# migoox/genome-downsampler

Hardware: AMD Instinct MI355X
Metric: Mreads/s selected at target coverage M=100 (higher is better)
Workload: dtype u32

## Files before the change

genome-downsampler_amd/csrc/api/context.inc.hip:

```cpp
namespace {

thread_local char g_err[512] = "";

int fail(int code, const char* fmt, ...) {
    va_list ap;
    va_start(ap, fmt);
    vsnprintf(g_err, sizeof(g_err), fmt, ap);
    va_end(ap);
    return code;
}

#define HIP_TRY(expr)                                                                      \
    do {                                                                                   \
        hipError_t _e = (expr);                                                            \
        if (_e != hipSuccess)                                                              \
            return fail(_e == hipErrorOutOfMemory ? QMCP_ENOMEM : QMCP_EHIP, "%s: %s (%s:%d)", \
                        #expr, hipGetErrorString(_e), __FILE__, __LINE__);                 \
    } while (0)

struct DevBuf {
    void* p = nullptr;
    size_t cap = 0;
};

// ... 21 lines not shown
    bool pm = false;
    uint32_t range_shift = 0;
    uint32_t nu_filter = 0;
};

}

struct qmcp_hip_ctx {
    int device = 0;
    qmcp_hip_options opt = {};
    hipStream_t stream = nullptr;
    hipEvent_t ev[EV_COUNT] = {};
    hipEvent_t ev_in = nullptr;
    hipStream_t stream2 = nullptr;
    hipEvent_t ev_fork = nullptr;
    DevBuf roff, poff, stats, cstart, boff, ecnt, eoff, selend, spine, hist, spine2, hist2, specsnap, specflags;
    DevBuf keys[2], vals[2];
    DevBuf in_starts, in_ends, in_aux0, in_aux1, mask, cov, amp, next_head;
    DevBuf f_starts, f_ends, f_map, f_words, f_mask;
    DevBuf ranges;
    DevBuf rankamb;
    DevBuf pm_desc, pm_work;
    uint32_t nu_ell = 0;
    uint64_t nu_failed_n = 0, nu_failed_ltot = 0;
    uint32_t nu_failed_ell = 0, nu_failed_M = 0;
    uint64_t nu_need_n = 0, nu_need_ltot = 0;
    uint32_t nu_need_ell = 0, nu_need_M = 0, nu_need_rounds = 0;
    bool nu_deferred = false;
    DevBuf nu_exc, nu_nadj, nu_ce, nu_state, nu_sus, nu_ckpt, nu_prev;
    uint32_t* h_nu = nullptr;
// ... 216 lines not shown
```

genome-downsampler_amd/csrc/api/host_entries.inc.hip:

```cpp
int coverage_common(qmcp_hip_ctx* c, const uint32_t* starts, const uint32_t* ends, uint64_t n64,
                    const uint64_t* roff, const uint32_t* lengths, uint32_t n_contigs,
                    const uint64_t* keep_mask, uint32_t* cov_out) {
    TRY(use_device(c));
    if (c->pending) return fail(QMCP_EINVAL, "a solve is pending on this context (call qmcp_hip_solve_end)");
    if (n64 && (!starts || !ends)) return fail(QMCP_EINVAL, "null buffer");
    Problem pr;
    TRY(check_problem(roff, lengths, n_contigs, n64, pr));
    const uint32_t n = (uint32_t)pr.n, ltot = (uint32_t)pr.ltot;
    if (ltot == 0) return n ? fail(QMCP_EREAD, "reads given for zero-length contigs") : QMCP_OK;
    if (n == 0) {
        if (cov_out) std::memset(cov_out, 0, (size_t)ltot * sizeof(uint32_t));
        TRY(ensure(c, c->cov, (size_t)ltot * sizeof(uint32_t)));
        HIP_TRY(hipMemsetAsync(c->cov.p, 0, (size_t)ltot * sizeof(uint32_t), c->stream));
        HIP_TRY(hipStreamSynchronize(c->stream));
        return QMCP_OK;
    }
    TRY(ensure(c, c->in_starts, (size_t)n * 4));
    TRY(ensure(c, c->in_ends, (size_t)n * 4));
    HIP_TRY(hipMemcpyAsync(c->in_starts.p, starts, (size_t)n * 4, hipMemcpyHostToDevice, c->stream));
    HIP_TRY(hipMemcpyAsync(c->in_ends.p, ends, (size_t)n * 4, hipMemcpyHostToDevice, c->stream));
    const uint64_t* d_keep = nullptr;
    if (keep_mask) {
        const size_t words = (size_t)((n64 + 63) / 64);
        TRY(ensure(c, c->mask, words * 8));
// ... 134 lines not shown
        if (b->p) (void)hipFree(b->p);
    for (int i = 0; i < EV_COUNT; ++i)
        if (c->ev[i]) (void)hipEventDestroy(c->ev[i]);
    if (c->ev_in) (void)hipEventDestroy(c->ev_in);
    for (auto& sp : c->spans) { (void)hipEventDestroy(sp.a); (void)hipEventDestroy(sp.b); }
    for (hipEvent_t e : c->ev_pool) (void)hipEventDestroy(e);
    if (c->h_tables) (void)hipHostFree(c->h_tables);
    if (c->h_scalars) (void)hipHostFree(c->h_scalars);
    if (c->h_stage) (void)hipHostFree(c->h_stage);
    if (c->h_mask) (void)hipHostFree(c->h_mask);
    for (hipEvent_t e : c->stage_ev) (void)hipEventDestroy(e);
    for (hipEvent_t e : c->stage_done) (void)hipEventDestroy(e);
    for (hipStream_t st : c->stage_streams) (void)hipStreamDestroy(st);
    if (c->ev_fork) (void)hipEventDestroy(c->ev_fork);
    if (c->ev_head) (void)hipEventDestroy(c->ev_head);
    if (c->ev_done) (void)hipEventDestroy(c->ev_done);
    if (c->h_head) (void)hipHostFree(c->h_head);
    if (c->h_nu) (void)hipHostFree(c->h_nu);
    if (c->stream2) (void)hipStreamDestroy(c->stream2);
    if (c->stream) (void)hipStreamDestroy(c->stream);
    delete c;
}

int qmcp_hip_set_profiling(qmcp_hip_ctx* c, int enabled) {
    if (!c) return fail(QMCP_EINVAL, "null context");
    c->profiling = enabled == 2 ? 2 : (enabled != 0 ? 1 : 0);
    c->acc.clear();
    return QMCP_OK;
}

// ... 494 lines not shown
```

genome-downsampler_amd/csrc/api/near_uniform_route.inc.hip:

```cpp
constexpr uint32_t kNuRunInsApart = 2;
int near_uniform_tail(qmcp_hip_ctx* c, uint32_t min_span, uint32_t max_span, uint32_t max_load, uint32_t* d_iters, bool& done) {
    done = false;
    SolveRun& run = c->run;
    const Problem& pr = run.pr;
    qmcp_hip_stats& local = run.local;
    const uint32_t n = (uint32_t)pr.n, ltot = (uint32_t)pr.ltot, n_contigs = run.n_contigs, M = run.M;
    local.near_uniform_giveup = QMCP_NU_GIVEUP_NOT_TRIED;
    if (c->opt.near_uniform < 0) return QMCP_OK;
    const uint32_t ell = max_span;
    uint32_t longest = 0;
    for (uint32_t k = 0; k < n_contigs; ++k) longest = run.lengths[k] > longest ? run.lengths[k] : longest;
    const qmcp::NearUniformPlan plan = qmcp::plan_near_uniform(c->opt, n, ell, min_span, ltot, n_contigs, longest, M, run.may_rank);
    const bool stretches = plan.stretches, speculate = plan.speculate;
    const bool dbg = c->opt.near_uniform_debug == 1;
    if (dbg) fprintf(stderr, "[near] pm %d may_rank %d ell %u ev %d depth %.2f min_span %u filter %u\n", (int)run.pm,
                     (int)run.may_rank, ell, (int)qmcp::sweep_uniform_ev_supported(ell, M), plan.depth, min_span, run.nu_filter);
    if (!plan.tried) return QMCP_OK;
    if (c->nu_failed_n == run.n64 && c->nu_failed_ltot == pr.ltot && c->nu_failed_ell == ell && c->nu_failed_M == M) {
        local.near_uniform_giveup = QMCP_NU_GIVEUP_REMEMBERED;
        c->nu_ell = 0;
        return QMCP_OK;
    }
    hipStream_t st = c->stream;
    const uint32_t cap = nu_cap_for(n);
// ... 10 lines not shown
        HIP_TRY(hipStreamSynchronize(st));
        n_exc = n - c->h_nu[0];
        if (dbg) fprintf(stderr, "[near] reads of span %u: %u of %u, list holds %u\n", ell, c->h_nu[0], n, cap);
        if (n_exc > n / 10u) {
            c->nu_ell = 0;
            local.near_uniform_giveup = n_exc > n - n / 10u ? QMCP_NU_GIVEUP_LONGER_READS : QMCP_NU_GIVEUP_TOO_MANY;
            return QMCP_OK;
        }
        c->nu_ell = ell;
        if (run.pm) TRY(queue_pm_head(c, st, ell));
        else TRY(queue_rm_head(c, st, ell, true));
        uint32_t* d_max_load = (uint32_t*)c->ranges.p + 65540;
        HIP_TRY(hipMemcpyAsync(c->h_nu, d_max_load, sizeof(uint32_t), hipMemcpyDeviceToHost, st));
        HIP_TRY(hipMemcpyAsync(c->h_nu + 1, d_stats + 4, 2 * sizeof(uint32_t), hipMemcpyDeviceToHost, st));
        HIP_TRY(hipStreamSynchronize(st));
        max_load = c->h_nu[0];
        if (c->h_nu[1] != n_exc || c->h_nu[2] != 0) { c->nu_ell = 0; local.near_uniform_giveup = QMCP_NU_GIVEUP_TOO_MANY; return QMCP_OK; }
    }
    local.near_uniform_exceptions = n_exc;
    if (n_exc == 0 || n_exc > n / 10u || (uint64_t)max_load * kRankBalance > (uint64_t)n) {
        if (n_exc > n / 10u) c->nu_ell = 0;
        local.near_uniform_giveup = n_exc > n / 10u ? QMCP_NU_GIVEUP_TOO_MANY : n_exc == 0 ? QMCP_NU_GIVEUP_NOT_TRIED : QMCP_NU_GIVEUP_HEAVY_RANGE;
        return QMCP_OK;
    }
    if (!stretches) {
        TRY(ensure(c, c->evpk, qmcp::sweep_ev_pack_bytes(ltot, ell, n_contigs + 768)));
        TRY(ensure(c, c->evlast, qmcp::sweep_ev_last_bytes(ltot, ell, n_contigs + 768)));
    }
    const uint32_t* boff = (const uint32_t*)c->boff.p;
    const uint64_t* poff = (const uint64_t*)c->poff.p;
// ... 150 lines not shown
```

genome-downsampler_amd/csrc/api/solve_head.inc.hip:

```cpp
int queue_rm_head(qmcp_hip_ctx* c, hipStream_t s1, uint32_t filter, bool clear_mask);
int queue_pm_head(qmcp_hip_ctx* c, hipStream_t st, uint32_t filter);

bool pm_route_ok(const qmcp_hip_ctx* c, const uint64_t* roff, const Problem& pr, uint32_t shift) {
    if (c->opt.pass_major < 0) return false;
    const uint32_t n = (uint32_t)pr.n, ltot = (uint32_t)pr.ltot;
    if ((uint64_t)qmcp::pm_slots(n, ltot, shift) >= (1ull << 31)) return false;
    if (c->opt.pass_major > 0) return true;
    double slots = 0.0;
    for (uint32_t k = 0; k < pr.n_contigs; ++k) {
        const uint64_t reads = roff[k + 1] - roff[k];
        if (reads == 0 || pr.poff[k + 1] == pr.poff[k]) continue;
        const double ranges = (double)(((pr.poff[k + 1] - 1) >> shift) - (pr.poff[k] >> shift) + 1);
        const double passes = (double)reads / (double)qmcp::pm_pass() < 1.0 ? 1.0 : (double)reads / (double)qmcp::pm_pass();
        const double slice = (double)reads / (passes * ranges);
        slots += passes * ranges * std::ceil(slice / 64.0);
    }
    return slots <= 1.3 * ((double)n / 64.0);
}
int enqueue_head(qmcp_hip_ctx* c, const uint32_t* d_starts, const uint32_t* d_ends,
                 const uint64_t* roff, const uint32_t* lengths, uint32_t n_contigs, uint64_t n64,
                 uint32_t M, uint64_t* d_mask) {
    if (c->pending) return fail(QMCP_EINVAL, "a solve is already pending on this context (call qmcp_hip_solve_end)");
    c->pend_spiky = false;
    if (!c->h_scalars) HIP_TRY(hipHostMalloc((void**)&c->h_scalars, 16 * sizeof(unsigned long long), hipHostMallocDefault));
    SolveRun& run = c->run;
    run = SolveRun();
    run.d_starts = d_starts; run.d_ends = d_ends; run.roff = roff; run.lengths = lengths;
    run.n_contigs = n_contigs; run.n64 = n64; run.M = M; run.d_mask = d_mask;
    Problem& pr = run.pr;
    TRY(check_problem(roff, lengths, n_contigs, n64, pr));
    const uint32_t n = (uint32_t)pr.n;
    const uint32_t ltot = (uint32_t)pr.ltot;
    const size_t mask_words = (size_t)((n64 + 63) / 64);
    qmcp_hip_stats& local = run.local;
    std::memset(&local, 0, sizeof(local));
    local.n_reads = n64;
    local.n_contigs = n_contigs;
    local.total_length = pr.ltot;
// ... 146 lines not shown
        qmcp::launch_partition_level2(s1, c->keys[1].p, n, range_shift, d_seg_tables, (uint32_t*)c->hist.p,
                                      (uint32_t*)c->spine.p, (uint16_t*)c->keys[0].p,
                                      (uint32_t*)c->vals[0].p, d_range_start, d_max_load);
    }
    HIP_TRY(hipEventRecord(c->ev_fork, s1));
    {
        KernelSpan sp(c, "k_range_offsets");
        qmcp::launch_range_offsets(s1, (const uint16_t*)c->keys[0].p, d_range_start, range_shift, ltot,
                                   (uint32_t*)c->boff.p, (uint32_t*)c->stats.p + 3);
    }
    HIP_TRY(hipGetLastError());
    run.nu_filter = filter;
    return QMCP_OK;
}

int queue_pm_head(qmcp_hip_ctx* c, hipStream_t st, uint32_t filter) {
    SolveRun& run = c->run;
    const uint32_t n = (uint32_t)run.pr.n, ltot = (uint32_t)run.pr.ltot, n_contigs = run.n_contigs;
    uint32_t* d_stats = (uint32_t*)c->stats.p;
    static const uint32_t zeros[4] = {0u, 0u, 0u, 0u};
    HIP_TRY(hipMemcpyAsync(d_stats + 3, zeros, sizeof(zeros), hipMemcpyHostToDevice, st));
    uint32_t* d_range_start = (uint32_t*)c->ranges.p;
    uint32_t* d_max_load = d_range_start + 65540;
    {
        KernelSpan sp(c, "k_pm_prepare_sort", st);
        qmcp::launch_pm_prepare_sort(st, run.d_starts, run.d_ends, n, (const uint64_t*)c->roff.p, (const uint64_t*)c->poff.p,
                                     n_contigs, run.range_shift, ltot, (uint16_t*)c->keys[0].p, (uint16_t*)c->keys[1].p,
                                     (uint32_t*)c->hist2.p, (uint32_t*)c->hist.p,
                                     (uint32_t*)c->pm_work.p, d_stats, (unsigned long long*)run.d_mask, filter,
                                     filter ? (uint32_t*)c->nu_exc.p : nullptr, nu_cap_for(n),
                                     filter ? qmcp::nu_exc_counts((uint32_t*)c->nu_exc.p, nu_cap_for(n)) : nullptr);
    }
    HIP_TRY(hipGetLastError());
    HIP_TRY(hipEventRecord(c->ev[EV_PREP], st));
    {
        KernelSpan sp(c, "scan_radix_hist(3 kernels)", st);
        qmcp::launch_exclusive_scan(st, (const uint32_t*)c->hist2.p, 256u * qmcp::pm_pitch(n), (uint32_t*)c->hist2.p,
                                    (uint32_t*)c->spine2.p, true);
    }
    {
        KernelSpan sp(c, "k_pm_descr + k_pm_range_table", st);
        qmcp::launch_pm_descr(st, (const uint32_t*)c->hist2.p, (const uint32_t*)c->hist.p, n, ltot, run.range_shift,
                              (uint32_t*)c->pm_desc.p, (uint32_t*)c->pm_work.p, d_range_start, d_max_load);
    }
    HIP_TRY(hipEventRecord(c->ev_fork, st));
    {
        KernelSpan sp(c, "k_pm_offsets", st);
        qmcp::launch_pm_offsets(st, (const uint16_t*)c->keys[0].p, (const uint32_t*)c->pm_desc.p, (const uint32_t*)c->hist2.p, n,
                                d_range_start, run.range_shift, ltot, (uint32_t*)c->boff.p, d_stats + 3);
    }
    HIP_TRY(hipGetLastError());
    run.nu_filter = filter;
    return QMCP_OK;
}

void queue_pm_rank(qmcp_hip_ctx* c, hipStream_t st, const uint32_t* ev_sev, const uint32_t* ev_lastns, uint32_t ell) {
    SolveRun& run = c->run;
    const uint32_t n = (uint32_t)run.pr.n, ltot = (uint32_t)run.pr.ltot;
    const bool by_records = qmcp::rank_scratch_by_records(run.range_shift, ltot, n);
    const uint16_t* keys16 = (const uint16_t*)c->keys[0].p;
    const uint16_t* idx16 = (const uint16_t*)c->keys[1].p;
    const uint32_t* desc = (const uint32_t*)c->pm_desc.p;
    const uint32_t* Tp = (const uint32_t*)c->hist2.p;
    const uint32_t* range_start = (const uint32_t*)c->ranges.p;
    uint32_t* amb_count = (uint32_t*)c->pm_work.p + 512;
    unsigned long long* kept_total = (unsigned long long*)c->scalars.p;
    {
        KernelSpan sp(c, "k_pm_walk", st);
        qmcp::launch_pm_walk(st, keys16, idx16, desc, Tp, n, range_start, run.range_shift, ltot, (const uint32_t*)c->boff.p,
                             (const uint32_t*)c->selend.p, (unsigned long long*)run.d_mask, kept_total, c->rankamb.p, by_records,
                             amb_count, ev_sev, ev_lastns, (const uint64_t*)c->poff.p, run.n_contigs, ell);
    }
    KernelSpan sp(c, "k_pm_settle", st);
    qmcp::launch_pm_settle(st, keys16, idx16, desc, Tp, n, range_start, run.range_shift, ltot, c->rankamb.p, by_records,
                           amb_count, (unsigned long long*)run.d_mask, kept_total);
}
```

genome-downsampler_amd/csrc/api/solve_tail.inc.hip:

```cpp
int enqueue_tail(qmcp_hip_ctx* c) {
    SolveRun& run = c->run;
    const Problem& pr = run.pr;
    qmcp_hip_stats& local = run.local;
    const uint32_t n = (uint32_t)pr.n, ltot = (uint32_t)pr.ltot, n_contigs = run.n_contigs, M = run.M;
    const uint64_t n64 = run.n64;
    const uint32_t *d_starts = run.d_starts, *d_ends = run.d_ends;
    uint64_t* const d_mask = run.d_mask;
    const uint64_t* roff = run.roff;
    const uint32_t* lengths = run.lengths;
    if (run.trivial) {
        for (int i = EV_PREP; i <= EV_MARK; ++i) HIP_TRY(hipEventRecord(c->ev[i], c->stream));
        for (int i = 0; i < 8; ++i) c->h_scalars[i] = 0;
        c->pend_stats = local;
        c->pend_whole_contig_chains = 0;
        c->pending = true;
        return QMCP_OK;
    }
    const uint32_t range_shift = run.range_shift;
    const bool may_rank = run.may_rank;
    uint32_t* d_range_start = (uint32_t*)c->ranges.p;
    const uint32_t* hs = c->h_head;
    bool have_gstart = run.have_gstart;
    const bool ranked_counted = run.ranked_counted;
    if (may_rank) {
// ... 30 lines not shown
        KernelSpan sp(c, "k_gstart");
        qmcp::launch_gstart(c->stream, d_starts, n, (const uint64_t*)c->roff.p, (const uint64_t*)c->poff.p,
                            n_contigs, (uint32_t*)c->vals[1].p);
        have_gstart = true;
    };
    bool sweep_done = false, ranked = false;
    uint32_t* d_iters = (uint32_t*)((char*)c->scalars.p + 16);
    bool near_done = false;
    uint32_t max_load_now = max_load;
    if (uniform && run.nu_filter != 0 && run.nu_filter != max_span) {
        c->nu_ell = 0;
        if (run.pm) TRY(queue_pm_head(c, c->stream, 0));
        else TRY(queue_rm_head(c, c->stream, 0, true));
        HIP_TRY(hipMemcpyAsync(c->h_nu, (uint32_t*)c->ranges.p + 65540, sizeof(uint32_t), hipMemcpyDeviceToHost, c->stream));
        HIP_TRY(hipStreamSynchronize(c->stream));
        max_load_now = c->h_nu[0];
    }
    if (!uniform) c->mixed_seen = true;
    if (!uniform && max_span <= qmcp::kMaxUniformSpan) {
        HIP_TRY(hipMemsetAsync(c->scalars.p, 0, 64, c->stream));
        TRY(near_uniform_tail(c, min_span, max_span, max_load, d_iters, near_done));
        if (near_done) {
            local.path = QMCP_PATH_NEAR_UNIFORM;
            sweep_done = ranked = true;
        }
    }
    if (!uniform && !near_done) {
        need_gstart();
        span_bits = bit_width(max_span - min_span);
        wide = pos_bits + span_bits > 32;
// ... 334 lines not shown
    qmcp_hip_ctx* c = new (std::nothrow) qmcp_hip_ctx();
    if (!c) return fail(QMCP_ENOMEM, "host allocation failed");
    c->device = device;
    qmcp_hip_default_options(&c->opt);
    options_from_env(c->opt);
    hipError_t e = hipStreamCreateWithFlags(&c->stream, hipStreamNonBlocking);
    for (int i = 0; e == hipSuccess && i < EV_COUNT; ++i) e = hipEventCreate(&c->ev[i]);
    if (e == hipSuccess) e = hipEventCreateWithFlags(&c->ev_in, hipEventDisableTiming);
    if (e == hipSuccess) {
        int lo = 0, hi = 0;
        (void)hipDeviceGetStreamPriorityRange(&lo, &hi);
        e = hipStreamCreateWithPriority(&c->stream2, hipStreamNonBlocking, hi);
    }
    if (e == hipSuccess) e = hipEventCreateWithFlags(&c->ev_fork, hipEventDisableTiming);
    if (e == hipSuccess) e = hipEventCreateWithFlags(&c->ev_head, hipEventDisableTiming);
    if (e == hipSuccess) e = hipEventCreateWithFlags(&c->ev_done, hipEventDisableTiming);
    if (e == hipSuccess) e = hipHostMalloc((void**)&c->h_head, 8 * sizeof(uint32_t), hipHostMallocDefault);
    if (e != hipSuccess) {
        qmcp_hip_destroy(c);
        return fail(QMCP_EHIP, "context setup: %s", hipGetErrorString(e));
    }
    *out_ctx = c;
    return QMCP_OK;
}


int solve_enqueue(qmcp_hip_ctx* c, const uint32_t* d_starts, const uint32_t* d_ends,
                  const uint64_t* roff, const uint32_t* lengths, uint32_t n_contigs, uint64_t n64,
                  uint32_t M, uint64_t* d_mask) {
    if (c->pending) return fail(QMCP_EINVAL, "a solve is already pending on this context (call qmcp_hip_solve_end)");
// ... 27 lines not shown
```

genome-downsampler_amd/csrc/kernels/pass_major.inc.hip:

```cpp
static constexpr int kPmPass = 8192;
__host__ __device__ inline uint32_t pm_stride_of(uint32_t n_ranges) { return (uint32_t)kPmPass + 64u * n_ranges; }
static constexpr int kPmThreads = 512;
static constexpr int kPmWaves = kPmThreads / 64;
static constexpr int kPmPassesPerWg = 4;
static constexpr size_t kPmSortLds = ((size_t)kPmPass + kPmWaves * 256 + 2 * 256 + 16 + 2 * kPmPassesPerWg * 256 + kPmWaves * 3 * 128) * sizeof(uint32_t);
static constexpr uint32_t kPmExcPerWave = 128;

#ifndef QMCP_PM_MIN_WAVES
#define QMCP_PM_MIN_WAVES 4
#endif
__global__ __launch_bounds__(kPmThreads, QMCP_PM_MIN_WAVES) void k_pm_prepare_sort(
    const uint32_t* __restrict__ starts, const uint32_t* __restrict__ ends, uint32_t n,
    const uint64_t* __restrict__ contig_read_off, const uint64_t* __restrict__ contig_pos_off, uint32_t n_contigs,
    uint32_t shift, uint32_t stride ,
    uint16_t* __restrict__ keys16, uint16_t* __restrict__ idx16,
    uint32_t* __restrict__ cnt_tab, uint32_t* __restrict__ lst_tab, uint32_t pitch ,
    uint32_t* __restrict__ work ,
    uint32_t* __restrict__ stats, unsigned long long* __restrict__ zero_mask,
    uint32_t ell_reg, uint32_t* __restrict__ exc, uint32_t exc_cap, uint32_t* __restrict__ exc_cnt) {
    extern __shared__ uint32_t s_pm[];
    uint32_t* s_stage = s_pm;
    uint32_t* s_cnt = s_stage + kPmPass;
    uint32_t* s_gbase = s_cnt + kPmWaves * 256;
    uint32_t* s_pbase = s_gbase + 256;
// ... 230 lines not shown
static constexpr uint32_t kPmWorkWords = 260;
static constexpr uint32_t kPmDescrY = 8;

struct PmSlot { uint32_t slot0, nv, pass; };
template <bool kVector>
__device__ __forceinline__ PmSlot pm_unpack(uint32_t dsc, bool has, uint32_t stride) {
    PmSlot s;
    s.pass = dsc >> 15;
    s.slot0 = has ? (kVector ? __umul24(s.pass, stride) : s.pass * stride) + (((dsc >> 6) & 511u) << 6) : 0u;
    s.nv = has ? (dsc & 63u) + 1u : 0u;
    return s;
}

__global__ __launch_bounds__(256) void k_pm_descr(const uint32_t* __restrict__ Tp, const uint32_t* __restrict__ lstw,
                                                  uint32_t pitch, uint32_t n_groups ,
                                                  uint32_t* __restrict__ desc, uint32_t* __restrict__ work) {
    __shared__ uint32_t s_red[4];
    const uint32_t d = blockIdx.x;
    const uint32_t per = (pitch + gridDim.y - 1u) / gridDim.y;
    const uint32_t P_end = min(pitch, (blockIdx.y + 1u) * per);
    uint32_t mine = 0;
    for (uint32_t P0 = blockIdx.y * per + threadIdx.x; P0 < P_end; P0 += 4u * 256u) {
        uint32_t w[4], t[4];
#pragma unroll
        for (int u = 0; u < 4; ++u) {
            const uint32_t P = min(P0 + (uint32_t)u * 256u, P_end - 1u);
            w[u] = lstw[(size_t)d * pitch + P];
            t[u] = Tp[(size_t)d * pitch + P];
        }
#pragma unroll
        for (int u = 0; u < 4; ++u) {
            const uint32_t P = P0 + (uint32_t)u * 256u;
            const uint32_t cnt = P < P_end ? w[u] >> 16 : 0u;
            if (cnt == 0u) continue;
            mine += cnt;
            const uint32_t g = t[u] >> 6;
            const uint32_t n_ws = (cnt + 63u) >> 6;
            for (uint32_t j = 0; j < n_ws; ++j)
                if (g + j < n_groups)
                    desc[g + j] = (P << 15) | (((w[u] & 0xFFFFu) + j) << 6) | (min(64u, cnt - 64u * j) - 1u);
        }
    }
    const uint32_t sum = wave_sum_u32(mine);
    if ((threadIdx.x & 63u) == 0u) s_red[threadIdx.x >> 6] = sum;
    __syncthreads();
    if (threadIdx.x == 0) {
        const uint32_t tot = s_red[0] + s_red[1] + s_red[2] + s_red[3];
        if (tot != 0u) atomicAdd(&work[d], tot);
    }
}

__global__ __launch_bounds__(256) void k_pm_range_table(const uint32_t* __restrict__ work, uint32_t* __restrict__ range_start,
                                                        uint32_t* __restrict__ max_load) {
    __shared__ uint32_t s_red[4];
    const uint32_t lane = threadIdx.x & 63u, wv = threadIdx.x >> 6;
    const uint32_t c = work[threadIdx.x];
    const uint32_t inc = wave_incl_scan_add(c);
    const uint32_t mx = wave_max_u32(c);
    if (lane == 63u) s_red[wv] = inc;
    __syncthreads();
    uint32_t base = 0;
    for (uint32_t x = 0; x < wv; ++x) base += s_red[x];
    range_start[threadIdx.x] = base + inc - c;
    if (threadIdx.x == 255u) range_start[256] = base + inc;
    __syncthreads();
    if (lane == 0u) s_red[wv] = mx;
    __syncthreads();
    if (threadIdx.x == 0) max_load[0] = max(max(s_red[0], s_red[1]), max(s_red[2], s_red[3]));
}

__global__ __launch_bounds__(1024) void k_pm_offsets(const uint16_t* __restrict__ keys16, const uint32_t* __restrict__ desc,
                                                     const uint32_t* __restrict__ Tp, uint32_t pitch,
                                                     const uint32_t* __restrict__ range_start ,
                                                     uint32_t shift, uint32_t stride, uint32_t ltot, uint32_t* __restrict__ boff,
                                                     uint32_t* __restrict__ empty_positions) {
    extern __shared__ uint32_t s_cnt32[];
#define PADDED(i) ((i) + ((i) >> 5))
    __shared__ uint32_t s_wsum[16], s_esum[16];
    const uint32_t range = blockIdx.x, width = 1u << shift, pos0 = range << shift;
    const uint32_t lo_p = Tp[(size_t)range * pitch], hi_p = Tp[(size_t)(range + 1) * pitch];
    const uint32_t g0 = lo_p >> 6, n_ws = (hi_p - lo_p) >> 6;
    const uint32_t lo = range_start[range];
    for (uint32_t i = threadIdx.x; i < width; i += blockDim.x) s_cnt32[PADDED(i)] = 0;
    __syncthreads();
    const uint32_t lane = threadIdx.x & 63u, nw = blockDim.x >> 6;
    const uint32_t w = (uint32_t)__builtin_amdgcn_readfirstlane((int)(threadIdx.x >> 6));
    const uint32_t sub = lane >> 4, l16 = lane & 15u;
    constexpr int kU = 4;
    const uint32_t n_quads = (n_ws + 3u) >> 2;
    for (uint32_t q0 = w; q0 < n_quads; q0 += kU * nw) {
        uint2 v[kU];
        uint32_t nv[kU];
#pragma unroll
        for (int u = 0; u < kU; ++u) {
            const uint32_t q = q0 + (uint32_t)u * nw;
            uint32_t dsc = 0;
            bool has = false;
            if (q < n_quads) {
                const uint32_t ws = 4u * q;
                const uint32_t d0 = desc[g0 + ws];
                const uint32_t d1 = ws + 1 < n_ws ? desc[g0 + ws + 1] : 0u;
                const uint32_t d2 = ws + 2 < n_ws ? desc[g0 + ws + 2] : 0u;
                const uint32_t d3 = ws + 3 < n_ws ? desc[g0 + ws + 3] : 0u;
                dsc = sub == 0 ? d0 : sub == 1 ? d1 : sub == 2 ? d2 : d3;
                has = ws + sub < n_ws;
            }
            const PmSlot at = pm_unpack<true>(dsc, has, stride);
            nv[u] = at.nv;
            v[u] = *reinterpret_cast<const uint2*>(keys16 + at.slot0 + 4u * l16);
        }
#pragma unroll
        for (int u = 0; u < kU; ++u) {
            const uint32_t e = 4u * l16;
            if (e < nv[u]) atomicAdd(&s_cnt32[PADDED(v[u].x & 0xFFFFu)], 1u);
            if (e + 1 < nv[u]) atomicAdd(&s_cnt32[PADDED(v[u].x >> 16)], 1u);
            if (e + 2 < nv[u]) atomicAdd(&s_cnt32[PADDED(v[u].y & 0xFFFFu)], 1u);
            if (e + 3 < nv[u]) atomicAdd(&s_cnt32[PADDED(v[u].y >> 16)], 1u);
        }
    }
    __syncthreads();
    const uint32_t per = width >= 1024u ? width >> 10 : 1u;
    const uint32_t firstp = threadIdx.x * per;
    uint32_t sum = 0, empties = 0;
    if (firstp < width)
        for (uint32_t qq = 0; qq < per; ++qq) {
            const uint32_t cq = s_cnt32[PADDED(firstp + qq)];
            sum += cq;
            empties += (cq == 0 && pos0 + firstp + qq < ltot) ? 1u : 0u;
        }
    const uint32_t inc = wave_incl_scan_add(sum);
    const uint32_t wv = threadIdx.x >> 6;
    if (lane == 63) s_wsum[wv] = inc;
// ... 287 lines not shown
uint32_t pm_exc_slots(uint32_t n) { return pm_pitch(n) * kPmWaves * kPmExcPerWave + kNuOverflow; }
void launch_pm_prepare_sort(hipStream_t st, const uint32_t* starts, const uint32_t* ends, uint32_t n,
                            const uint64_t* d_roff, const uint64_t* d_poff, uint32_t n_contigs, uint32_t shift, uint32_t ltot,
                            uint16_t* keys16, uint16_t* idx16, uint32_t* cnt_tab, uint32_t* lst_tab,
                            uint32_t* work, uint32_t* stats, unsigned long long* zero_mask, uint32_t ell_reg, uint32_t* exc,
                            uint32_t exc_cap, uint32_t* exc_cnt) {
    const uint32_t pitch = pm_pitch(n);
    if (pitch == 0) return;
    (void)hipFuncSetAttribute((const void*)k_pm_prepare_sort, hipFuncAttributeMaxDynamicSharedMemorySize, (int)kPmSortLds);
    hipLaunchKernelGGL(k_pm_prepare_sort, dim3(pitch / kPmPassesPerWg), dim3(kPmThreads), kPmSortLds, st, starts, ends, n,
                       d_roff, d_poff, n_contigs, shift, pm_stride(ltot, shift), keys16, idx16, cnt_tab, lst_tab, pitch,
                       work, stats, zero_mask, exc != nullptr ? ell_reg : 0u, exc, exc_cap, exc_cnt);
    if (exc != nullptr && ell_reg != 0u)
        hipLaunchKernelGGL(k_nu_count_groups, dim3(32), dim3(256), 0, st, exc_cnt, pitch * kPmWaves, stats);
}
void launch_pm_descr(hipStream_t st, const uint32_t* Tp, const uint32_t* lstw, uint32_t n, uint32_t ltot, uint32_t shift,
                     uint32_t* desc, uint32_t* work, uint32_t* range_start, uint32_t* max_load) {
    const uint32_t pitch = pm_pitch(n), n_ranges = (ltot >> shift) + 1u;
    const uint32_t s64 = pm_stride(ltot, shift) / 64u;
    hipLaunchKernelGGL(k_pm_descr, dim3(n_ranges, kPmDescrY), dim3(256), 0, st, Tp, lstw, pitch, pitch * s64, desc, work);
    hipLaunchKernelGGL(k_pm_range_table, dim3(1), dim3(256), 0, st, work, range_start, max_load);
}
void launch_pm_offsets(hipStream_t st, const uint16_t* keys16, const uint32_t* desc, const uint32_t* Tp, uint32_t n,
                       const uint32_t* range_start, uint32_t shift, uint32_t ltot, uint32_t* boff, uint32_t* empty_positions) {
    const uint32_t n_ranges = (ltot >> shift) + 1;
    const size_t width = (size_t)1 << shift;
    const size_t lds = (width + width / 32 + 1) * sizeof(uint32_t);
    (void)hipFuncSetAttribute((const void*)k_pm_offsets, hipFuncAttributeMaxDynamicSharedMemorySize, (int)lds);
    hipLaunchKernelGGL(k_pm_offsets, dim3(n_ranges), dim3(1024), lds, st, keys16, desc, Tp, pm_pitch(n), range_start, shift,
                       pm_stride(ltot, shift), ltot, boff, empty_positions);
}
void launch_pm_walk(hipStream_t st, const uint16_t* keys16, const uint16_t* idx16, const uint32_t* desc, const uint32_t* Tp,
                    uint32_t n, const uint32_t* range_start, uint32_t shift, uint32_t ltot, const uint32_t* boff,
                    const uint32_t* selend, unsigned long long* mask, unsigned long long* kept_total, void* scratch,
                    bool scratch_by_records, uint32_t* amb_count, const uint32_t* ev_sev, const uint32_t* ev_lastns,
                    const uint64_t* d_poff, uint32_t n_contigs, uint32_t ell) {
    const uint32_t n_ranges = (ltot >> shift) + 1;
    const EvQuota evq{ev_sev, ev_lastns, d_poff, n_contigs, ell};
    const size_t lds = (((size_t)1 << shift) + 1) * sizeof(uint32_t);
    (void)hipFuncSetAttribute((const void*)k_pm_walk, hipFuncAttributeMaxDynamicSharedMemorySize, (int)lds);
    hipLaunchKernelGGL(k_pm_walk, dim3(n_ranges), dim3(1024), lds, st, keys16, idx16, desc, Tp, pm_pitch(n), range_start, shift,
                       pm_stride(ltot, shift), ltot, boff, selend, evq, mask, (uint2*)scratch, scratch_by_records ? 1 : 0,
                       amb_count, kept_total);
}
void launch_pm_settle(hipStream_t st, const uint16_t* keys16, const uint16_t* idx16, const uint32_t* desc, const uint32_t* Tp,
// ... 9 lines not shown
```

genome-downsampler_amd/csrc/qmcp_kernels.h:

```cpp
#ifndef QMCP_KERNELS_H
#define QMCP_KERNELS_H
#include <hip/hip_runtime.h>
#include <stdint.h>

#include "sweep_plan.h"

namespace qmcp {

static constexpr uint32_t kMaxLdsRingSpan = 16383;
static constexpr uint32_t kMaxGeneralSpan = (1u << 24) - 1;
static constexpr uint32_t kMaxUniformSpan = 512;
static constexpr uint32_t kMaxCachedSpan = 4032;

void launch_prepare(hipStream_t st, const uint32_t* starts, const uint32_t* ends, uint32_t n,
                    const uint64_t* d_roff, const uint64_t* d_poff, uint32_t n_contigs,
                    const uint64_t* keep_mask, uint32_t* gstart, uint32_t* cstart,
                    uint32_t* stats, uint32_t part_shift,
                    uint32_t* part_hist ,
                    uint32_t* digit0_hist ,
                    uint32_t* global_digit_hist ,
                    unsigned long long* zero_mask ,
                    uint32_t ell_reg = 0, uint32_t* exc = nullptr, uint32_t exc_cap = 0, uint32_t* exc_cnt = nullptr
                    );
uint32_t prepare_exc_slots(uint32_t n);
// ... 133 lines not shown
                      const uint32_t* selend, unsigned long long* mask, unsigned long long* kept_total,
                      void* scratch, bool scratch_by_records);

uint32_t pm_pitch(uint32_t n);
uint32_t pm_pass();
uint32_t pm_stride(uint32_t ltot, uint32_t shift);
size_t pm_slots(uint32_t n, uint32_t ltot, uint32_t shift);
uint32_t pm_work_words();
void launch_pm_prepare_sort(hipStream_t st, const uint32_t* starts, const uint32_t* ends, uint32_t n,
                            const uint64_t* d_roff, const uint64_t* d_poff, uint32_t n_contigs, uint32_t shift, uint32_t ltot,
                            uint16_t* keys16, uint16_t* idx16, uint32_t* cnt_tab, uint32_t* lst_tab,
                            uint32_t* work ,
                            uint32_t* stats, unsigned long long* zero_mask, uint32_t ell_reg = 0, uint32_t* exc = nullptr,
                            uint32_t exc_cap = 0, uint32_t* exc_cnt = nullptr);
uint32_t pm_exc_slots(uint32_t n);
void launch_pm_descr(hipStream_t st, const uint32_t* Tp, const uint32_t* lstw, uint32_t n, uint32_t ltot, uint32_t shift,
                     uint32_t* desc, uint32_t* work, uint32_t* range_start, uint32_t* max_load);
void launch_pm_offsets(hipStream_t st, const uint16_t* keys16, const uint32_t* desc, const uint32_t* Tp, uint32_t n,
                       const uint32_t* range_start, uint32_t shift, uint32_t ltot, uint32_t* boff, uint32_t* empty_positions);
void launch_pm_walk(hipStream_t st, const uint16_t* keys16, const uint16_t* idx16, const uint32_t* desc, const uint32_t* Tp,
                    uint32_t n, const uint32_t* range_start, uint32_t shift, uint32_t ltot, const uint32_t* boff,
                    const uint32_t* selend, unsigned long long* mask, unsigned long long* kept_total, void* scratch,
                    bool scratch_by_records, uint32_t* amb_count,
                    const uint32_t* ev_sev = nullptr, const uint32_t* ev_lastns = nullptr,
                    const uint64_t* d_poff = nullptr, uint32_t n_contigs = 0, uint32_t ell = 0);
void launch_pm_settle(hipStream_t st, const uint16_t* keys16, const uint16_t* idx16, const uint32_t* desc, const uint32_t* Tp,
                      uint32_t n, const uint32_t* range_start, uint32_t shift, uint32_t ltot, const void* scratch,
                      bool scratch_by_records, const uint32_t* amb_count, unsigned long long* mask,
                      unsigned long long* kept_total);


void launch_span_mode_share(hipStream_t st, const uint32_t* starts, const uint32_t* ends, uint32_t n, uint32_t* out );
size_t nu_exc_bytes(uint32_t cap);
// ... 76 lines not shown
```

Measured before the change: 117,300.

## Move pass-major scan and descriptor build to side stream, derive offsets from row tables

Splits k_pm_descr so per-range totals and occupied-block spans come from a new k_pm_row_totals kernel on the main stream, while the exclusive scan and descriptor build run on stream2 and overlap with k_pm_offsets. k_pm_offsets now reconstructs warp-slot positions directly from the per-row count table with wave scans and readlanes, so it no longer needs the descriptor array, and it keeps more loads in flight. The walk waits on an event for the descriptor tables, and extra stream2 synchronizations are added at host sync points. This removes the scan and descriptor work from the critical path at the cost of more in-kernel index reconstruction and cross-stream ordering complexity.

```diff
diff --git a/genome-downsampler_amd/csrc/api/context.inc.hip b/genome-downsampler_amd/csrc/api/context.inc.hip
--- a/genome-downsampler_amd/csrc/api/context.inc.hip
+++ b/genome-downsampler_amd/csrc/api/context.inc.hip
@@ -59,6 +59,8 @@
     hipEvent_t ev_in = nullptr;
     hipStream_t stream2 = nullptr;
     hipEvent_t ev_fork = nullptr;
+    hipEvent_t ev_prod = nullptr, ev_tables = nullptr;
+    bool pm_tables_on_side = false;
     DevBuf roff, poff, stats, cstart, boff, ecnt, eoff, selend, spine, hist, spine2, hist2, specsnap, specflags;
     DevBuf keys[2], vals[2];
     DevBuf in_starts, in_ends, in_aux0, in_aux1, mask, cov, amp, next_head;
diff --git a/genome-downsampler_amd/csrc/api/host_entries.inc.hip b/genome-downsampler_amd/csrc/api/host_entries.inc.hip
--- a/genome-downsampler_amd/csrc/api/host_entries.inc.hip
+++ b/genome-downsampler_amd/csrc/api/host_entries.inc.hip
@@ -172,6 +172,8 @@
     for (hipStream_t st : c->stage_streams) (void)hipStreamDestroy(st);
     if (c->ev_fork) (void)hipEventDestroy(c->ev_fork);
     if (c->ev_head) (void)hipEventDestroy(c->ev_head);
+    if (c->ev_prod) (void)hipEventDestroy(c->ev_prod);
+    if (c->ev_tables) (void)hipEventDestroy(c->ev_tables);
     if (c->ev_done) (void)hipEventDestroy(c->ev_done);
     if (c->h_head) (void)hipHostFree(c->h_head);
     if (c->h_nu) (void)hipHostFree(c->h_nu);
diff --git a/genome-downsampler_amd/csrc/api/near_uniform_route.inc.hip b/genome-downsampler_amd/csrc/api/near_uniform_route.inc.hip
--- a/genome-downsampler_amd/csrc/api/near_uniform_route.inc.hip
+++ b/genome-downsampler_amd/csrc/api/near_uniform_route.inc.hip
@@ -48,6 +48,7 @@
         HIP_TRY(hipMemcpyAsync(c->h_nu, d_max_load, sizeof(uint32_t), hipMemcpyDeviceToHost, st));
         HIP_TRY(hipMemcpyAsync(c->h_nu + 1, d_stats + 4, 2 * sizeof(uint32_t), hipMemcpyDeviceToHost, st));
         HIP_TRY(hipStreamSynchronize(st));
+        HIP_TRY(hipStreamSynchronize(c->stream2));
         max_load = c->h_nu[0];
         if (c->h_nu[1] != n_exc || c->h_nu[2] != 0) { c->nu_ell = 0; local.near_uniform_giveup = QMCP_NU_GIVEUP_TOO_MANY; return QMCP_OK; }
     }
diff --git a/genome-downsampler_amd/csrc/api/solve_head.inc.hip b/genome-downsampler_amd/csrc/api/solve_head.inc.hip
--- a/genome-downsampler_amd/csrc/api/solve_head.inc.hip
+++ b/genome-downsampler_amd/csrc/api/solve_head.inc.hip
@@ -22,6 +22,7 @@
                  uint32_t M, uint64_t* d_mask) {
     if (c->pending) return fail(QMCP_EINVAL, "a solve is already pending on this context (call qmcp_hip_solve_end)");
     c->pend_spiky = false;
+    c->pm_tables_on_side = false;
     if (!c->h_scalars) HIP_TRY(hipHostMalloc((void**)&c->h_scalars, 16 * sizeof(unsigned long long), hipHostMallocDefault));
     SolveRun& run = c->run;
     run = SolveRun();
@@ -198,6 +199,9 @@
     return QMCP_OK;
 }
 
+#ifndef QMCP_PM_TABLES_ON_SIDE_STREAM
+#define QMCP_PM_TABLES_ON_SIDE_STREAM 1
+#endif
 int queue_pm_head(qmcp_hip_ctx* c, hipStream_t st, uint32_t filter) {
     SolveRun& run = c->run;
     const uint32_t n = (uint32_t)run.pr.n, ltot = (uint32_t)run.pr.ltot, n_contigs = run.n_contigs;
@@ -206,6 +210,7 @@
     HIP_TRY(hipMemcpyAsync(d_stats + 3, zeros, sizeof(zeros), hipMemcpyHostToDevice, st));
     uint32_t* d_range_start = (uint32_t*)c->ranges.p;
     uint32_t* d_max_load = d_range_start + 65540;
+    uint32_t* d_row_span = (uint32_t*)c->pm_work.p + 768;
     {
         KernelSpan sp(c, "k_pm_prepare_sort", st);
         qmcp::launch_pm_prepare_sort(st, run.d_starts, run.d_ends, n, (const uint64_t*)c->roff.p, (const uint64_t*)c->poff.p,
@@ -217,22 +222,36 @@
     }
     HIP_TRY(hipGetLastError());
     HIP_TRY(hipEventRecord(c->ev[EV_PREP], st));
-    {
-        KernelSpan sp(c, "scan_radix_hist(3 kernels)", st);
-        qmcp::launch_exclusive_scan(st, (const uint32_t*)c->hist2.p, 256u * qmcp::pm_pitch(n), (uint32_t*)c->hist2.p,
-                                    (uint32_t*)c->spine2.p, true);
+    auto queue_tables = [&](hipStream_t ts) {
+        {
+            KernelSpan sp(c, "scan_radix_hist(3 kernels)", ts);
+            qmcp::launch_exclusive_scan(ts, (const uint32_t*)c->hist2.p, 256u * qmcp::pm_pitch(n), (uint32_t*)c->hist2.p,
+                                        (uint32_t*)c->spine2.p, true);
+        }
+        KernelSpan sp(c, "k_pm_descr + k_pm_range_table", ts);
+        qmcp::launch_pm_descr(ts, (const uint32_t*)c->hist2.p, (const uint32_t*)c->hist.p, n, ltot, run.range_shift,
+                              (uint32_t*)c->pm_desc.p);
+    };
+    const bool side = QMCP_PM_TABLES_ON_SIDE_STREAM != 0;
+    if (side) {
+        HIP_TRY(hipEventRecord(c->ev_prod, st));
+        HIP_TRY(hipStreamWaitEvent(c->stream2, c->ev_prod, 0));
+        queue_tables(c->stream2);
+        HIP_TRY(hipEventRecord(c->ev_tables, c->stream2));
+        c->pm_tables_on_side = true;
     }
     {
         KernelSpan sp(c, "k_pm_descr + k_pm_range_table", st);
-        qmcp::launch_pm_descr(st, (const uint32_t*)c->hist2.p, (const uint32_t*)c->hist.p, n, ltot, run.range_shift,
-                              (uint32_t*)c->pm_desc.p, (uint32_t*)c->pm_work.p, d_range_start, d_max_load);
+        qmcp::launch_pm_row_totals(st, (const uint32_t*)c->hist.p, n, ltot, run.range_shift, (uint32_t*)c->pm_work.p, d_row_span,
+                                   d_range_start, d_max_load);
     }
     HIP_TRY(hipEventRecord(c->ev_fork, st));
     {
         KernelSpan sp(c, "k_pm_offsets", st);
-        qmcp::launch_pm_offsets(st, (const uint16_t*)c->keys[0].p, (const uint32_t*)c->pm_desc.p, (const uint32_t*)c->hist2.p, n,
+        qmcp::launch_pm_offsets(st, (const uint16_t*)c->keys[0].p, (const uint32_t*)c->hist.p, d_row_span, n,
                                 d_range_start, run.range_shift, ltot, (uint32_t*)c->boff.p, d_stats + 3);
     }
+    if (!side) queue_tables(st);
     HIP_TRY(hipGetLastError());
     run.nu_filter = filter;
     return QMCP_OK;
@@ -249,6 +268,10 @@
     const uint32_t* range_start = (const uint32_t*)c->ranges.p;
     uint32_t* amb_count = (uint32_t*)c->pm_work.p + 512;
     unsigned long long* kept_total = (unsigned long long*)c->scalars.p;
+    if (c->pm_tables_on_side) {
+        (void)hipStreamWaitEvent(st, c->ev_tables, 0);
+        c->pm_tables_on_side = false;
+    }
     {
         KernelSpan sp(c, "k_pm_walk", st);
         qmcp::launch_pm_walk(st, keys16, idx16, desc, Tp, n, range_start, run.range_shift, ltot, (const uint32_t*)c->boff.p,
diff --git a/genome-downsampler_amd/csrc/api/solve_tail.inc.hip b/genome-downsampler_amd/csrc/api/solve_tail.inc.hip
--- a/genome-downsampler_amd/csrc/api/solve_tail.inc.hip
+++ b/genome-downsampler_amd/csrc/api/solve_tail.inc.hip
@@ -68,6 +68,7 @@
         else TRY(queue_rm_head(c, c->stream, 0, true));
         HIP_TRY(hipMemcpyAsync(c->h_nu, (uint32_t*)c->ranges.p + 65540, sizeof(uint32_t), hipMemcpyDeviceToHost, c->stream));
         HIP_TRY(hipStreamSynchronize(c->stream));
+        HIP_TRY(hipStreamSynchronize(c->stream2));
         max_load_now = c->h_nu[0];
     }
     if (!uniform) c->mixed_seen = true;
@@ -432,6 +433,8 @@
     }
     if (e == hipSuccess) e = hipEventCreateWithFlags(&c->ev_fork, hipEventDisableTiming);
     if (e == hipSuccess) e = hipEventCreateWithFlags(&c->ev_head, hipEventDisableTiming);
+    if (e == hipSuccess) e = hipEventCreateWithFlags(&c->ev_prod, hipEventDisableTiming);
+    if (e == hipSuccess) e = hipEventCreateWithFlags(&c->ev_tables, hipEventDisableTiming);
     if (e == hipSuccess) e = hipEventCreateWithFlags(&c->ev_done, hipEventDisableTiming);
     if (e == hipSuccess) e = hipHostMalloc((void**)&c->h_head, 8 * sizeof(uint32_t), hipHostMallocDefault);
     if (e != hipSuccess) {
diff --git a/genome-downsampler_amd/csrc/kernels/pass_major.inc.hip b/genome-downsampler_amd/csrc/kernels/pass_major.inc.hip
--- a/genome-downsampler_amd/csrc/kernels/pass_major.inc.hip
+++ b/genome-downsampler_amd/csrc/kernels/pass_major.inc.hip
@@ -268,12 +268,10 @@
 
 __global__ __launch_bounds__(256) void k_pm_descr(const uint32_t* __restrict__ Tp, const uint32_t* __restrict__ lstw,
                                                   uint32_t pitch, uint32_t n_groups ,
-                                                  uint32_t* __restrict__ desc, uint32_t* __restrict__ work) {
-    __shared__ uint32_t s_red[4];
+                                                  uint32_t* __restrict__ desc) {
     const uint32_t d = blockIdx.x;
     const uint32_t per = (pitch + gridDim.y - 1u) / gridDim.y;
     const uint32_t P_end = min(pitch, (blockIdx.y + 1u) * per);
-    uint32_t mine = 0;
     for (uint32_t P0 = blockIdx.y * per + threadIdx.x; P0 < P_end; P0 += 4u * 256u) {
         uint32_t w[4], t[4];
 #pragma unroll
@@ -287,7 +285,6 @@
             const uint32_t P = P0 + (uint32_t)u * 256u;
             const uint32_t cnt = P < P_end ? w[u] >> 16 : 0u;
             if (cnt == 0u) continue;
-            mine += cnt;
             const uint32_t g = t[u] >> 6;
             const uint32_t n_ws = (cnt + 63u) >> 6;
             for (uint32_t j = 0; j < n_ws; ++j)
@@ -295,12 +292,42 @@
                     desc[g + j] = (P << 15) | (((w[u] & 0xFFFFu) + j) << 6) | (min(64u, cnt - 64u * j) - 1u);
         }
     }
-    const uint32_t sum = wave_sum_u32(mine);
-    if ((threadIdx.x & 63u) == 0u) s_red[threadIdx.x >> 6] = sum;
+}
+
+static constexpr uint32_t kPmRowThreads = 1024;
+__global__ __launch_bounds__(kPmRowThreads) void k_pm_row_totals(const uint32_t* __restrict__ lstw, uint32_t pitch ,
+                                                                uint32_t* __restrict__ work, uint32_t* __restrict__ row_span) {
+    __shared__ uint32_t s_red[3][kPmRowThreads / 64];
+    const uint32_t d = blockIdx.x;
+    const uint4* const row = reinterpret_cast<const uint4*>(lstw + (size_t)d * pitch);
+    const uint32_t quads = pitch >> 2;
+    uint32_t sum = 0, first = 0xFFFFFFFFu, end = 0;
+    constexpr int kU = 4;
+    for (uint32_t q0 = threadIdx.x; q0 < quads; q0 += kU * kPmRowThreads) {
+        uint4 e[kU];
+#pragma unroll
+        for (int u = 0; u < kU; ++u) e[u] = row[min(q0 + (uint32_t)u * kPmRowThreads, quads - 1u)];
+#pragma unroll
+        for (int u = 0; u < kU; ++u) {
+            const uint32_t q = q0 + (uint32_t)u * kPmRowThreads;
+            const uint32_t c = (e[u].x >> 16) + (e[u].y >> 16) + (e[u].z >> 16) + (e[u].w >> 16);
+            if (q < quads && c != 0u) {
+                sum += c;
+                first = min(first, 4u * q);
+                end = max(end, 4u * q + 4u);
+            }
+        }
+    }
+    sum = wave_sum_u32(sum);
+    first = wave_min_u32(first);
+    end = wave_max_u32(end);
+    const uint32_t lane = threadIdx.x & 63u, wv = threadIdx.x >> 6;
+    if (lane == 0u) { s_red[0][wv] = sum; s_red[1][wv] = first; s_red[2][wv] = end; }
     __syncthreads();
     if (threadIdx.x == 0) {
-        const uint32_t tot = s_red[0] + s_red[1] + s_red[2] + s_red[3];
-        if (tot != 0u) atomicAdd(&work[d], tot);
+        for (uint32_t x = 1; x < kPmRowThreads / 64; ++x) { sum += s_red[0][x]; first = min(first, s_red[1][x]); end = max(end, s_red[2][x]); }
+        work[d] = sum;
+        row_span[d] = end != 0u ? (first >> 6) | (((end + 63u) >> 6) << 16) : 0u;
     }
 }
 
@@ -323,53 +350,76 @@
     if (threadIdx.x == 0) max_load[0] = max(max(s_red[0], s_red[1]), max(s_red[2], s_red[3]));
 }
 
-__global__ __launch_bounds__(1024) void k_pm_offsets(const uint16_t* __restrict__ keys16, const uint32_t* __restrict__ desc,
-                                                     const uint32_t* __restrict__ Tp, uint32_t pitch,
-                                                     const uint32_t* __restrict__ range_start ,
-                                                     uint32_t shift, uint32_t stride, uint32_t ltot, uint32_t* __restrict__ boff,
-                                                     uint32_t* __restrict__ empty_positions) {
+static constexpr int kPmOffDepth = 10;
+static constexpr uint32_t kPmOffShare = 4;
+static constexpr uint32_t kPmOffWaves = 16;
+__global__ __launch_bounds__(64 * kPmOffWaves) void k_pm_offsets(const uint16_t* __restrict__ keys16, const uint32_t* __restrict__ lst_tab,
+                                                                 uint32_t pitch, const uint32_t* __restrict__ row_span,
+                                                                 const uint32_t* __restrict__ range_start ,
+                                                                 uint32_t shift, uint32_t stride, uint32_t ltot, uint32_t* __restrict__ boff,
+                                                                 uint32_t* __restrict__ empty_positions) {
     extern __shared__ uint32_t s_cnt32[];
 #define PADDED(i) ((i) + ((i) >> 5))
     __shared__ uint32_t s_wsum[16], s_esum[16];
     const uint32_t range = blockIdx.x, width = 1u << shift, pos0 = range << shift;
-    const uint32_t lo_p = Tp[(size_t)range * pitch], hi_p = Tp[(size_t)(range + 1) * pitch];
-    const uint32_t g0 = lo_p >> 6, n_ws = (hi_p - lo_p) >> 6;
     const uint32_t lo = range_start[range];
     for (uint32_t i = threadIdx.x; i < width; i += blockDim.x) s_cnt32[PADDED(i)] = 0;
     __syncthreads();
     const uint32_t lane = threadIdx.x & 63u, nw = blockDim.x >> 6;
     const uint32_t w = (uint32_t)__builtin_amdgcn_readfirstlane((int)(threadIdx.x >> 6));
     const uint32_t sub = lane >> 4, l16 = lane & 15u;
-    constexpr int kU = 4;
-    const uint32_t n_quads = (n_ws + 3u) >> 2;
-    for (uint32_t q0 = w; q0 < n_quads; q0 += kU * nw) {
-        uint2 v[kU];
-        uint32_t nv[kU];
-#pragma unroll
-        for (int u = 0; u < kU; ++u) {
-            const uint32_t q = q0 + (uint32_t)u * nw;
-            uint32_t dsc = 0;
-            bool has = false;
-            if (q < n_quads) {
-                const uint32_t ws = 4u * q;
-                const uint32_t d0 = desc[g0 + ws];
-                const uint32_t d1 = ws + 1 < n_ws ? desc[g0 + ws + 1] : 0u;
-                const uint32_t d2 = ws + 2 < n_ws ? desc[g0 + ws + 2] : 0u;
-                const uint32_t d3 = ws + 3 < n_ws ? desc[g0 + ws + 3] : 0u;
-                dsc = sub == 0 ? d0 : sub == 1 ? d1 : sub == 2 ? d2 : d3;
-                has = ws + sub < n_ws;
-            }
-            const PmSlot at = pm_unpack<true>(dsc, has, stride);
-            nv[u] = at.nv;
-            v[u] = *reinterpret_cast<const uint2*>(keys16 + at.slot0 + 4u * l16);
-        }
-#pragma unroll
-        for (int u = 0; u < kU; ++u) {
-            const uint32_t e = 4u * l16;
-            if (e < nv[u]) atomicAdd(&s_cnt32[PADDED(v[u].x & 0xFFFFu)], 1u);
-            if (e + 1 < nv[u]) atomicAdd(&s_cnt32[PADDED(v[u].x >> 16)], 1u);
-            if (e + 2 < nv[u]) atomicAdd(&s_cnt32[PADDED(v[u].y & 0xFFFFu)], 1u);
-            if (e + 3 < nv[u]) atomicAdd(&s_cnt32[PADDED(v[u].y >> 16)], 1u);
+    {
+        const uint32_t* const row = lst_tab + (size_t)range * pitch;
+        const uint32_t span = (uint32_t)__builtin_amdgcn_readfirstlane((int)row_span[range]);
+        const uint32_t b_end = span >> 16;
+        const uint32_t mem = w % kPmOffShare;
+        constexpr uint32_t kGroups = kPmOffWaves / kPmOffShare;
+        auto entries_of = [&](uint32_t blk) -> uint32_t {
+            const uint32_t P = blk * 64u + lane;
+            return (blk < b_end && P < pitch) ? row[P] : 0u;
+        };
+        uint32_t blk = (span & 0xFFFFu) + w / kPmOffShare;
+        uint32_t ent_next = entries_of(blk);
+        uint32_t r_before = 0;
+        for (; blk < b_end; blk += kGroups) {
+            const uint32_t ent = ent_next;
+            ent_next = entries_of(blk + kGroups);
+            const uint32_t mine = ((ent >> 16) + 63u) >> 6;
+            const uint32_t incl = wave_incl_scan_add(mine);
+            const uint32_t n_ws = (uint32_t)__builtin_amdgcn_readlane((int)incl, 63);
+            const uint32_t n_req = (n_ws + 3u) >> 2;
+            const uint32_t P0 = blk * 64u;
+            for (uint32_t r0 = (mem - r_before) & (kPmOffShare - 1u); r0 < n_req; r0 += kPmOffDepth * kPmOffShare) {
+                uint2 v[kPmOffDepth];
+                uint32_t nv[kPmOffDepth];
+#pragma unroll
+                for (int u = 0; u < kPmOffDepth; ++u) {
+                    const uint32_t k0 = 4u * (r0 + (uint32_t)u * kPmOffShare);
+                    uint32_t e = 0, upto = 0, j = 0;
+#pragma unroll
+                    for (uint32_t x = 0; x < 4u; ++x) {
+                        const uint32_t jx = min(63u, (uint32_t)__popcll(__ballot(incl <= k0 + x)));
+                        const uint32_t ex = (uint32_t)__builtin_amdgcn_readlane((int)ent, (int)jx);
+                        const uint32_t ix = (uint32_t)__builtin_amdgcn_readlane((int)incl, (int)jx);
+                        if (sub == x) { e = ex; upto = ix; j = jx; }
+                    }
+                    const bool has = k0 + sub < n_ws;
+                    const uint32_t cnt = e >> 16;
+                    const uint32_t t = k0 + sub + ((cnt + 63u) >> 6) - upto;
+                    nv[u] = has ? min(64u, cnt - 64u * t) : 0u;
+                    const uint32_t slot0 = has ? __umul24(P0 + j, stride) + (((e & 0xFFFFu) + t) << 6) : 0u;
+                    v[u] = *reinterpret_cast<const uint2*>(keys16 + slot0 + 4u * l16);
+                }
+#pragma unroll
+                for (int u = 0; u < kPmOffDepth; ++u) {
+                    const uint32_t e = 4u * l16;
+                    if (e < nv[u]) atomicAdd(&s_cnt32[PADDED(v[u].x & 0xFFFFu)], 1u);
+                    if (e + 1 < nv[u]) atomicAdd(&s_cnt32[PADDED(v[u].x >> 16)], 1u);
+                    if (e + 2 < nv[u]) atomicAdd(&s_cnt32[PADDED(v[u].y & 0xFFFFu)], 1u);
+                    if (e + 3 < nv[u]) atomicAdd(&s_cnt32[PADDED(v[u].y >> 16)], 1u);
+                }
+            }
+            r_before += n_req;
         }
     }
     __syncthreads();
@@ -687,21 +737,26 @@
     if (exc != nullptr && ell_reg != 0u)
         hipLaunchKernelGGL(k_nu_count_groups, dim3(32), dim3(256), 0, st, exc_cnt, pitch * kPmWaves, stats);
 }
+void launch_pm_row_totals(hipStream_t st, const uint32_t* lstw, uint32_t n, uint32_t ltot, uint32_t shift, uint32_t* work,
+                          uint32_t* row_span, uint32_t* range_start, uint32_t* max_load) {
+    const uint32_t n_ranges = (ltot >> shift) + 1u;
+    hipLaunchKernelGGL(k_pm_row_totals, dim3(n_ranges), dim3(kPmRowThreads), 0, st, lstw, pm_pitch(n), work, row_span);
+    hipLaunchKernelGGL(k_pm_range_table, dim3(1), dim3(256), 0, st, work, range_start, max_load);
+}
 void launch_pm_descr(hipStream_t st, const uint32_t* Tp, const uint32_t* lstw, uint32_t n, uint32_t ltot, uint32_t shift,
-                     uint32_t* desc, uint32_t* work, uint32_t* range_start, uint32_t* max_load) {
+                     uint32_t* desc) {
     const uint32_t pitch = pm_pitch(n), n_ranges = (ltot >> shift) + 1u;
     const uint32_t s64 = pm_stride(ltot, shift) / 64u;
-    hipLaunchKernelGGL(k_pm_descr, dim3(n_ranges, kPmDescrY), dim3(256), 0, st, Tp, lstw, pitch, pitch * s64, desc, work);
-    hipLaunchKernelGGL(k_pm_range_table, dim3(1), dim3(256), 0, st, work, range_start, max_load);
-}
-void launch_pm_offsets(hipStream_t st, const uint16_t* keys16, const uint32_t* desc, const uint32_t* Tp, uint32_t n,
+    hipLaunchKernelGGL(k_pm_descr, dim3(n_ranges, kPmDescrY), dim3(256), 0, st, Tp, lstw, pitch, pitch * s64, desc);
+}
+void launch_pm_offsets(hipStream_t st, const uint16_t* keys16, const uint32_t* lstw, const uint32_t* row_span, uint32_t n,
                        const uint32_t* range_start, uint32_t shift, uint32_t ltot, uint32_t* boff, uint32_t* empty_positions) {
     const uint32_t n_ranges = (ltot >> shift) + 1;
     const size_t width = (size_t)1 << shift;
     const size_t lds = (width + width / 32 + 1) * sizeof(uint32_t);
     (void)hipFuncSetAttribute((const void*)k_pm_offsets, hipFuncAttributeMaxDynamicSharedMemorySize, (int)lds);
-    hipLaunchKernelGGL(k_pm_offsets, dim3(n_ranges), dim3(1024), lds, st, keys16, desc, Tp, pm_pitch(n), range_start, shift,
-                       pm_stride(ltot, shift), ltot, boff, empty_positions);
+    hipLaunchKernelGGL(k_pm_offsets, dim3(n_ranges), dim3(64 * kPmOffWaves), lds, st, keys16, lstw, pm_pitch(n), row_span,
+                       range_start, shift, pm_stride(ltot, shift), ltot, boff, empty_positions);
 }
 void launch_pm_walk(hipStream_t st, const uint16_t* keys16, const uint16_t* idx16, const uint32_t* desc, const uint32_t* Tp,
                     uint32_t n, const uint32_t* range_start, uint32_t shift, uint32_t ltot, const uint32_t* boff,
diff --git a/genome-downsampler_amd/csrc/qmcp_kernels.h b/genome-downsampler_amd/csrc/qmcp_kernels.h
--- a/genome-downsampler_amd/csrc/qmcp_kernels.h
+++ b/genome-downsampler_amd/csrc/qmcp_kernels.h
@@ -171,9 +171,11 @@
                             uint32_t* stats, unsigned long long* zero_mask, uint32_t ell_reg = 0, uint32_t* exc = nullptr,
                             uint32_t exc_cap = 0, uint32_t* exc_cnt = nullptr);
 uint32_t pm_exc_slots(uint32_t n);
+void launch_pm_row_totals(hipStream_t st, const uint32_t* lstw, uint32_t n, uint32_t ltot, uint32_t shift, uint32_t* work,
+                          uint32_t* row_span, uint32_t* range_start, uint32_t* max_load);
 void launch_pm_descr(hipStream_t st, const uint32_t* Tp, const uint32_t* lstw, uint32_t n, uint32_t ltot, uint32_t shift,
-                     uint32_t* desc, uint32_t* work, uint32_t* range_start, uint32_t* max_load);
-void launch_pm_offsets(hipStream_t st, const uint16_t* keys16, const uint32_t* desc, const uint32_t* Tp, uint32_t n,
+                     uint32_t* desc);
+void launch_pm_offsets(hipStream_t st, const uint16_t* keys16, const uint32_t* lstw, const uint32_t* row_span, uint32_t n,
                        const uint32_t* range_start, uint32_t shift, uint32_t ltot, uint32_t* boff, uint32_t* empty_positions);
 void launch_pm_walk(hipStream_t st, const uint16_t* keys16, const uint16_t* idx16, const uint32_t* desc, const uint32_t* Tp,
                     uint32_t n, const uint32_t* range_start, uint32_t shift, uint32_t ltot, const uint32_t* boff,
```

Result: no change. 117,100 (-0.1%).
